# malak29/video-text-detection-system

Measured on AMD Instinct MI355X. Metric: frames/sec (detect+recognize) @720p, 1/2/4/8 MI355X; box IoU vs CPU ref, higher is better.
Workload: dtype f16

## Files before the change

video-text-detection-system_amd/csrc/vtd_api.cpp:

```cpp
#include <algorithm>
#include <cmath>
#include <cstdio>
#include <cstdlib>
#include <cstring>
#include <map>
#include <memory>
#include <string>
#include <vector>

#include "../../include/vtd.h"
#include "vtd_common.h"

int vtd_launch_conv(const ConvParams& p, int cfg, hipStream_t stream);
int vtd_conv_num_configs();
bool vtd_conv_config_valid(const ConvParams& p, int cfg);
int vtd_launch_preprocess(const uint8_t* frames, int n, int H, int W, half_t* out, const int* xb, const int* xk, int ksx,
                          const int* yb, const int* yk, int ksy, int max_rows, hipStream_t stream);
int vtd_launch_nchw_to_input(const float* x, half_t* out, int n, hipStream_t stream);
int vtd_launch_maxpool(const TensorDesc& in, const TensorDesc& out, int n, int kh, int kw, int sh, int sw, int pad_h, int pad_w,
                       hipStream_t stream);
void vtd_stem_pool_pack_weights(const float* w_folded, half_t* packed);
int vtd_launch_stem_pool(const TensorDesc& in, const TensorDesc& out, const half_t* w_packed, const float* bias, int n, hipStream_t stream);
extern "C" int vtd_head_entry_halo_steps(int py, int px, int nch1, int* out);
int vtd_launch_head_entry_halo(const ConvParams& c, const int* steps_dev, int nsteps, int big_tiles, hipStream_t stream);
#ifdef VTD_EXPERIMENTAL_CANDIDATES
extern "C" int vtd_head_entry_half_schedule(const int* steps, int nsteps, int* out);
int vtd_launch_head_entry_half(const ConvParams& c, const int* sched_dev, int nsteps, hipStream_t stream);
int vtd_head_entry_pair_tables(int py, int px, int c2ch, int* half_steps, int* plan);
int vtd_launch_head_entry_pair(const ConvParams& c, const int* half_steps_dev, const int* plan_dev, int nh, hipStream_t stream);
#endif
bool vtd_conv_halo_supported(const ConvParams& c, int* bn_out, int* tw_out);
bool vtd_conv_halo_c64_supported(const ConvParams& c, int tw);
int vtd_launch_conv_halo(const ConvParams& c, int bn, int tw, hipStream_t stream);
bool vtd_pointwise128_supported(const ConvParams& c);
int vtd_launch_pointwise128(const ConvParams& c, hipStream_t stream);
void vtd_head_tail_pack_w1(const half_t* w1_gemm, half_t* packed);
void vtd_head_tail_pack_w2(const float* w2, half_t* packed);
int vtd_launch_head_tail(const TensorDesc& in, const half_t* w1, const float* bias1, const half_t* w2, float b2, float* out, int n,
                         hipStream_t stream);

int vtd_launch_crop_resize(const uint8_t* frames, int H, int W, const int32_t* boxes, int ncrops, uint8_t* out, hipStream_t s);
int vtd_launch_crnn_conv1(const uint8_t* in_u8, const float* in_f32, const half_t* w, const float* bias, half_t* out, int n, hipStream_t s);
int vtd_launch_lstm(const half_t* xs, const half_t* whh, half_t* hout, int D, int T, hipStream_t s);
int vtd_launch_ctc_greedy(const float* logits, int n, int T, int V, int ld, const int32_t* id2char, int blank, int apply_softmax,
                          int32_t* out, hipStream_t s);
int vtd_launch_compact_rows(const float* in, float* out, int64_t rows, int V, int ld, hipStream_t s);
int vtd_dbloss_ws_bytes();
int vtd_launch_dbloss(const float* prob, const float* thresh, const float* prob_t, const float* thresh_t, int64_t n, float smooth, double* workspace,
                      float* out4, double* sums5, hipStream_t stream);
int vtd_launch_dbloss_backward(const float* prob, const float* thresh, const float* prob_t, const float* thresh_t, int64_t n, float smooth,
                               const double* sums5, const float* grad_out4, float* grad_prob, float* grad_thresh, hipStream_t stream);
int vtd_launch_binary_counts(const float* pred, const float* target, int64_t n, float threshold, int64_t* counts4, hipStream_t stream);
int64_t vtd_dbhead_ws_bytes(int n, int H, int W, int backward);
int vtd_launch_dbhead_pack(const void* x, int dtype, int n, int H, int W, void* feats, hipStream_t s);
int vtd_launch_dbhead_forward(const void* feats, int n, int H, int W, const vtd_dbhead_params* params, int training, float momentum, float eps,
                              void* ws, float* prob, float* thresh, float* stats_out, hipStream_t s);
int vtd_launch_dbhead_backward_input(int n, int H, int W, const vtd_dbhead_params* params, void* scratch, float* dfeats, float* dscale, hipStream_t s);
int vtd_launch_dbhead_unpack_input_grad(const float* dfeats, const float* dscale, int n, int H, int W, float* out, hipStream_t s);
int vtd_launch_dbhead_backward(const void* feats, int n, int H, int W, const vtd_dbhead_params* params, int training, const void* ws,
                               const float* prob, const float* thresh, const float* gprob, const float* gthresh, const vtd_dbhead_params* grads,
                               void* scratch, hipStream_t s);

namespace vtd {

enum : int {
    ERR_ARG = -1100,
    ERR_UNKNOWN_KEY = -1101,
    ERR_SHAPE = -1102,
    ERR_MISSING_KEY = -1103,
    ERR_NOT_FINALIZED = -1104,
    ERR_BATCH = -1105,
    ERR_GEOMETRY = -1106,
    ERR_CAPACITY = -1107,
};

using StateDict = std::map<std::string, std::vector<float>>;

struct DeviceArena {
    std::vector<void*> blocks;
    size_t total = 0;
    int alloc(void** out, size_t bytes, bool zero) {
        void* p = nullptr;
        bytes = (bytes + 255) & ~size_t(255);
        hipError_t e = hipMalloc(&p, bytes);
        if (e != hipSuccess) return -(int)e;
        if (zero) {
            e = hipMemset(p, 0, bytes);
            if (e != hipSuccess) return -(int)e;
// ... 6 lines not shown
    ~DeviceArena() {
        for (void* p : blocks) (void)hipFree(p);
    }
};

static TensorDesc make_desc(int n, int h, int w, int c, int ring, int ring_br) {
    TensorDesc t;
    t.ptr = nullptr;
    t.n = n; t.h = h; t.w = w; t.c = c; t.ring = ring;
    t.hp = h + ring + ring_br;
    t.wp = w + ring + ring_br;
    return t;
}

struct ConvOp {
    TensorDesc in, out, res;
    bool has_res = false;
    half_t* w = nullptr;
    half_t* w_panel = nullptr;
    float* bias = nullptr;
    int k_hi_step = 32, cin_steps = 1, kw = 1, s_step = 0, r_step = 0;
    int K = 0, cout = 0, cout_pad = 0, stride = 1, in_y0 = 0, in_x0 = 0, flags = 0, ps_cout = 0, res_shift = 0;
    int ho = 0, wo = 0;
    int64_t macs_per_image = 0;
    void* out_f32 = nullptr;
    int ldc = 0;
    int seg_cols = 0;
    void* seg_out[3] = {nullptr, nullptr, nullptr};
    int seg_ldc[3] = {0, 0, 0};
    const float* head_w = nullptr;
    float head_b = 0.f;
    const uint32_t* plist = nullptr;
    const int* tile_combo = nullptr;
    const uint32_t* plist_b = nullptr;
    const int* tile_combo_border = nullptr;
    int tiles_border = 0;
    const int* he_steps = nullptr;
    int he_nsteps = 0;
    const int* hh_sched = nullptr;
    const int* hp_half_steps = nullptr;
    const int* hp_plan = nullptr;
    int hp_nh = 0;
    const int* tile_combo_b = nullptr;
    int tiles_per_img_b = 0;
    int tiles_per_img = 0, seg1_steps = 0, cin_steps2 = 0, kw2 = 0, s_step2 = 0, r_step2 = 0, img_h = 0, img_w = 0;
    TensorDesc in2;
    const float* bias_tab = nullptr;
    bool dual = false;
    int in2_mul = 1, in2_shr = 0;
    int pool_pw = 0;
};

struct Op {
    enum Kind { CONV, POOL, FINAL, STEMPOOL, HEADTAIL, BORDER } kind;
    ConvOp conv;
    TensorDesc pin, pout;
    int pk[6] = {0, 0, 0, 0, 0, 0};
    const float* fw = nullptr;
    float fbias = 0.f;
    int final_slot = 0;
    const half_t* spw = nullptr;
    const float* spb = nullptr;
    const half_t* htw1 = nullptr;
    const half_t* htw2 = nullptr;
};

static void fill_conv_params(const ConvOp& c, int n, ConvParams& p) {
    std::memset(&p, 0, sizeof(p));
    p.in = c.in.ptr; p.wgt = c.w; p.k_hi_step = c.k_hi_step; p.cin_steps = c.cin_steps; p.kw = c.kw; p.s_step = c.s_step; p.r_step = c.r_step; p.bias = c.bias;
    p.res = c.has_res ? c.res.ptr : nullptr;
    p.out = (c.flags & (EPI_OUT_F32 | EPI_OUT_F16)) ? c.out_f32 : (void*)c.out.ptr;
    p.M = n * c.ho * c.wo; p.K = c.K; p.cout = c.cout; p.cout_pad = c.cout_pad;
    p.ho = c.ho; p.wo = c.wo;
    p.in_hp = c.in.hp; p.in_wp = c.in.wp; p.in_c = c.in.c; p.in_y0 = c.in_y0; p.in_x0 = c.in_x0; p.stride = c.stride;
    p.out_hp = c.out.hp; p.out_wp = c.out.wp; p.out_c = c.out.c; p.out_ring = c.out.ring;
    p.res_hp = c.res.hp; p.res_wp = c.res.wp; p.res_ring = c.res.ring; p.res_shift = c.res_shift;
    p.ps_cout = c.ps_cout; p.flags = c.flags; p.ldc = c.ldc;
    p.seg_cols = c.seg_cols;
    for (int i = 0; i < 3; ++i) { p.seg_out[i] = c.seg_out[i]; p.seg_ldc[i] = c.seg_ldc[i]; }
    p.head_w = c.head_w; p.head_b = c.head_b; p.prob_out = (float*)c.out_f32;
    if (c.plist) {
        p.plist = c.plist; p.tile_combo = c.tile_combo; p.tiles_per_img = c.tiles_per_img;
        p.plist_b = c.plist_b; p.tile_combo_b = c.tile_combo_b; p.tiles_per_img_b = c.tiles_per_img_b;
        p.in2 = c.in2.ptr; p.in2_hp = c.in2.hp; p.in2_wp = c.in2.wp; p.in2_c = c.in2.c; p.in2_ring = c.in2.ring;
        p.seg1_steps = c.seg1_steps; p.cin_steps2 = c.cin_steps2; p.kw2 = c.kw2; p.s_step2 = c.s_step2; p.r_step2 = c.r_step2;
        p.bias_tab = c.bias_tab; p.img_h = c.img_h; p.img_w = c.img_w;
        p.M = n * c.tiles_per_img * 128;
    }
    p.pool_pw = c.pool_pw;
    if (c.dual) {
        p.in2 = c.in2.ptr; p.in2_hp = c.in2.hp; p.in2_wp = c.in2.wp; p.in2_c = c.in2.c; p.in2_ring = c.in2.ring;
        p.in2_mul = c.in2_mul; p.in2_shr = c.in2_shr;
        p.seg1_steps = c.seg1_steps; p.cin_steps2 = c.cin_steps2; p.kw2 = 1; p.s_step2 = 0; p.r_step2 = 0;
    }
}

static const int kHaloCfg = 100;
static const int kHaloC64Cfg = 101;
static const int kHalo64Cfg = 104;
static const int kHeadEntryHalo256Cfg = 103;
static const int kHeadEntryPairCfg = 105;
static const int kPointwiseCfg = 106;
static const int kHeadEntryHalfCfg = 107;
static const int kHeadEntryHaloCfg = 102;
static bool halo_enabled() {
    const char* e = std::getenv("VTD_HALO_CONV");
    return !(e && e[0] == '0');
}

static int pick_tile_height(const ConvParams& p, int table_cfg) {
    if (const char* e = std::getenv("VTD_TILE_HEIGHT_MODEL"); e && e[0] == '0') return table_cfg;
    if (std::getenv("VTD_FORCE_CONV_CFG")) return table_cfg;
    static const struct { int cfg, bm, bn; double eff; } family[5] = {{0, 256, 128, 1.0}, {14, 256, 128, 1.04}, {13, 272, 128, 0.92}, {12, 208, 128, 0.80},
                                                                      {15, 256, 256, 1.07}};
    auto cost_of = [&](int cfg) -> double {
        for (const auto& k : family)
            if (k.cfg == cfg) {
                if (!vtd_conv_config_valid(p, k.cfg)) return 0.0;
                const int64_t tiles = (int64_t)((p.M + k.bm - 1) / k.bm) * (p.cout_pad / k.bn);
                return (double)((tiles + 255) / 256) * k.bm * k.bn / k.eff;
            }
        return 0.0;
    };
    int best = table_cfg;
    double best_cost = cost_of(table_cfg);
    if (best_cost == 0.0) return table_cfg;
    const double keep = best_cost * 0.94;
    double other_cost = keep;
    for (const auto& k : family) {
        if (k.cfg == table_cfg) continue;
        const double c = cost_of(k.cfg);
        if (c > 0.0 && c < other_cost) { other_cost = c; best = k.cfg; }
    }
    (void)best_cost;
    return best;
}

static int launch_conv_op(const ConvOp& c, int n, hipStream_t s, int cfg = -1, float* prob_out = nullptr) {
    ConvParams p;
    fill_conv_params(c, n, p);
    if (prob_out) p.prob_out = prob_out;
#ifdef VTD_EXPERIMENTAL_CANDIDATES
    if (cfg == kHeadEntryPairCfg) {
        if (!c.hp_half_steps || !c.tile_combo_border) return ERR_GEOMETRY;
        return vtd_launch_head_entry_pair(p, c.hp_half_steps, c.hp_plan, c.hp_nh, s);
    }
    if (cfg == kHeadEntryHalfCfg) {
        if (!c.hh_sched || !c.tile_combo_border) return ERR_GEOMETRY;
        return vtd_launch_head_entry_half(p, c.hh_sched, c.he_nsteps, s);
    }
#else
    if (cfg == kHeadEntryPairCfg || cfg == kHeadEntryHalfCfg) return ERR_GEOMETRY;
#endif
    if (cfg == kHeadEntryHaloCfg || cfg == kHeadEntryHalo256Cfg) {
        if (!c.he_steps || !c.tile_combo_border) return ERR_GEOMETRY;
        return vtd_launch_head_entry_halo(p, c.he_steps, c.he_nsteps, cfg == kHeadEntryHalo256Cfg ? 1 : 0, s);
// ... 238 lines not shown
    const char* p = text;
    while (*p) {
        const char* eol = std::strchr(p, '\n');
        std::string line = eol ? std::string(p, eol) : std::string(p);
        p = eol ? eol + 1 : p + line.size();
        if (line.empty() || line[0] == '#') continue;
        const size_t sp = line.find_last_of(" \t");
        if (sp == std::string::npos || sp + 1 >= line.size()) return ERR_ARG;
        char* end = nullptr;
        const long v = std::strtol(line.c_str() + sp + 1, &end, 10);
        if (!end || *end != 0) return ERR_ARG;
        size_t ke = sp;
        while (ke > 0 && (line[ke - 1] == ' ' || line[ke - 1] == '\t')) --ke;
        m->tuning[line.substr(0, ke)] = (int)v;
    }
    return 0;
}

static int64_t get_tuning_text(const ModelBase* m, char* buf, int64_t cap) {
    if (!m) return ERR_ARG;
    std::string out;
    for (const auto& kv : m->tuning) out += kv.first + " " + std::to_string(kv.second) + "\n";
    if (buf && cap > 0) {
        const size_t ncopy = std::min((size_t)cap - 1, out.size());
        std::memcpy(buf, out.data(), ncopy);
        buf[ncopy] = 0;
    }
    return (int64_t)out.size() + 1;
}

static int batch_bucket(int n, int cap) {
    int b = 1;
    while (b < n) b <<= 1;
    return std::min(b, cap);
}

}

struct vtd_detector : vtd::ModelBase {
    std::string backbone;
    int max_batch = 0;
    bool finalized = false;
    std::vector<Op> ops;
    TensorDesc input;
    std::map<std::string, TensorDesc> taps;
    std::map<std::pair<int, int>, PreTables> pre;
    int64_t macs = 0;
    float* final_out[2] = {nullptr, nullptr};
    std::map<int, std::vector<int>> tuned;
    bool head_tail_kernel = true;
    bool fuse_stem_pool = true;
    bool fuse_fpn_head = true;
    bool fuse_downsample = true;
    size_t p2_ops = 0;
    bool profiling = false;
    int prof_only = -1;
    std::vector<hipEvent_t> ev_pool;
    size_t ev_used = 0;
    std::vector<std::pair<int, std::pair<hipEvent_t, hipEvent_t>>> ev_spans;
    std::vector<double> prof_ms;
    std::vector<int64_t> prof_calls;
    std::vector<double> prof_macs;
    hipEvent_t take_event() {
        if (ev_used == ev_pool.size()) {
            hipEvent_t e;
            if (hipEventCreate(&e) != hipSuccess) return nullptr;
            ev_pool.push_back(e);
        }
        return ev_pool[ev_used++];
    }
    ~vtd_detector() {
        for (hipEvent_t e : ev_pool) (void)hipEventDestroy(e);
    }
};


struct vtd_recognizer : vtd::ModelBase {
    int vocab = 0, max_crops = 0;
    bool finalized = false;
    bool fuse_pools = true;
    uint8_t* resized = nullptr;
    half_t* w1 = nullptr;
    float* b1 = nullptr;
    TensorDesc t1;
    std::vector<Op> ops;
    TensorDesc t7, h0, h1;
    ConvOp xs_gemm[2], cls_gemm;
    half_t* whh[2] = {nullptr, nullptr};
    half_t* xs = nullptr;
    float* logits_pad = nullptr;
    std::map<std::string, TensorDesc> taps;
    int64_t macs = 0;
    std::map<int, std::vector<int>> tuned;
};

namespace vtd {

struct Fold {
    std::vector<double> scale, shift;
};

static inline half_t half_of(double v) {
    volatile float f = (float)v;
    return (half_t)f;
}

// ... 489 lines not shown
                TensorDesc t1;
                if ((rc = new_tensor(hout, hout, width, t1))) return rc;
                Fold f1, f2;
                if ((rc = fold_bn(d, pre + ".bn1", "", width, f1))) return rc;
                ConvOp c1;
                if ((rc = build_conv(d, c1, x, t1, pre + ".conv1.weight", f1, cin, width, 3, 3, stride, 1, EPI_RELU))) return rc;
                push_conv(c1);
                if ((rc = new_tensor(hout, hout, width, y, (fuse && st == 0 && b == counts[st] - 1) ? 2 : 1))) return rc;
                if ((rc = fold_bn(d, pre + ".bn2", "", width, f2))) return rc;
                ConvOp c2;
                HostConv h2;
                h2.host_only = fold_ds;
                if ((rc = build_conv(d, c2, t1, y, pre + ".conv2.weight", f2, width, width, 3, 3, 1, 1, fold_ds ? EPI_RELU : (EPI_RELU | EPI_RESIDUAL), &h2))) return rc;
                if (fold_ds) {
                    if ((rc = attach_second_segment(d, c2, h2, ds_op, ds_host, stride, 0))) return rc;
                } else {
                    c2.has_res = true; c2.res = idt; c2.res_shift = 0;
                }
                push_conv(c2);
            } else {
                TensorDesc t1, t2;
                if ((rc = new_tensor(hin, hin, width, t1))) return rc;
                Fold f1, f2, f3;
                if ((rc = fold_bn(d, pre + ".bn1", "", width, f1))) return rc;
                ConvOp c1;
                if ((rc = build_conv(d, c1, x, t1, pre + ".conv1.weight", f1, cin, width, 1, 1, 1, 0, EPI_RELU))) return rc;
                push_conv(c1);
                if ((rc = new_tensor(hout, hout, width, t2))) return rc;
                if ((rc = fold_bn(d, pre + ".bn2", "", width, f2))) return rc;
                ConvOp c2;
                if ((rc = build_conv(d, c2, t1, t2, pre + ".conv2.weight", f2, width, width, 3, 3, stride, 1, EPI_RELU))) return rc;
                push_conv(c2);
                if ((rc = new_tensor(hout, hout, cout, y, (fuse && st == 0 && b == counts[st] - 1) ? 2 : 1))) return rc;
                if ((rc = fold_bn(d, pre + ".bn3", "", cout, f3))) return rc;
                ConvOp c3;
                HostConv h3;
                h3.host_only = fold_ds;
                if ((rc = build_conv(d, c3, t2, y, pre + ".conv3.weight", f3, width, cout, 1, 1, 1, 0, fold_ds ? EPI_RELU : (EPI_RELU | EPI_RESIDUAL), &h3))) return rc;
                if (fold_ds) {
                    if ((rc = attach_second_segment(d, c3, h3, ds_op, ds_host, stride, 0))) return rc;
                } else {
                    c3.has_res = true; c3.res = idt; c3.res_shift = 0;
                }
                push_conv(c3);
            }
            x = y;
            cin = cout;
        }
        tapsC[st] = x;
        d->taps["c" + std::to_string(st + 2)] = x;
    }

    TensorDesc last;
    for (int i = 0; i < (fuse ? 3 : 4); ++i) {
        const TensorDesc& feat = tapsC[3 - i];
        TensorDesc lat;
        if ((rc = new_tensor(feat.h, feat.w, 256, lat))) return rc;
        Fold f;
        const std::string k = "fpn.inner_blocks." + std::to_string(i);
        if ((rc = fold_bn(d, "", k + ".bias", 256, f))) return rc;
        ConvOp c;
        if ((rc = build_conv(d, c, feat, lat, k + ".weight", f, feat.c, 256, 1, 1, 1, 0, i ? EPI_RESIDUAL : 0))) return rc;
        if (i) { c.has_res = true; c.res = last; c.res_shift = 1; }
        push_conv(c);
        last = lat;
    }
    TensorDesc p2;
    if (!fuse) {
        if ((rc = new_tensor(160, 160, 256, p2))) return rc;
        Fold f;
        if ((rc = fold_bn(d, "", "fpn.layer_blocks.3.bias", 256, f))) return rc;
        ConvOp c;
        if ((rc = build_conv(d, c, last, p2, "fpn.layer_blocks.3.weight", f, 256, 256, 3, 3, 1, 1, 0))) return rc;
        push_conv(c);
        d->taps["p2"] = p2;
        d->p2_ops = d->ops.size();
    } else if (!d->get("fpn.inner_blocks.3.weight", (size_t)256 * tapsC[0].c) || !d->get("fpn.layer_blocks.3.weight", (size_t)256 * 256 * 9)) {
        return ERR_MISSING_KEY;
    }
    for (int i = 0; i < 3; ++i) {
        const std::string k = "fpn.layer_blocks." + std::to_string(i);
        if (!d->get(k + ".weight", (size_t)256 * 256 * 9) || !d->get(k + ".bias", 256)) return ERR_MISSING_KEY;
    }

    const char* branch[2] = {"head.probability_head.", "head.threshold_head."};
    for (int br = 0; br < 2; ++br) {
        const std::string hp = branch[br];
        TensorDesc h1;
        if ((rc = new_tensor(160, 160, 64, h1))) return rc;
        Fold f1, f2;
        ConvOp c1;
        if (fuse) {
            if ((rc = build_classed_head_entry(d, c1, tapsC[0], last, h1, hp))) return rc;
        } else {
            if ((rc = fold_bn(d, hp + "1", hp + "0.bias", 64, f1))) return rc;
            if ((rc = build_conv(d, c1, p2, h1, hp + "0.weight", f1, 256, 64, 3, 3, 1, 1, EPI_RELU))) return rc;
        }
        if ((rc = fold_bn(d, hp + "4", hp + "3.bias", 64, f2))) return rc;
        ConvOp c2;
        TensorDesc h2 = make_desc(B, 320, 320, 64, 1, 1);
        std::vector<half_t> w1_host;
        if ((rc = build_convt(d, c2, h1, h2, hp + "3.weight", f2, 64, 64, EPI_RELU, &w1_host))) return rc;
        auto w6 = d->get(hp + "6.weight", 64 * 4), b6 = d->get(hp + "6.bias", 1);
        if (!w6 || !b6) return ERR_MISSING_KEY;
        std::vector<float> wf(4 * 64);
        for (int blk = 0; blk < 4; ++blk)
            for (int ci = 0; ci < 64; ++ci) wf[blk * 64 + ci] = (*w6)[ci * 4 + blk];
        float* wdev = nullptr;
        if ((rc = upload(d->arena, wf.data(), wf.size() * sizeof(float), (void**)&wdev))) return rc;
        c2.flags = EPI_HEAD_FINAL;
        c2.head_w = wdev;
        c2.head_b = (*b6)[0];
        Op o1, o2;
        o1.kind = Op::CONV; o1.conv = c1; o1.final_slot = br;
        o2.kind = Op::FINAL; o2.conv = c2; o2.final_slot = br;
        if (d->head_tail_kernel) {
            std::vector<half_t> p1((size_t)4 * 4 * 2 * 64 * 8), p2((size_t)2 * 64 * 8);
            vtd_head_tail_pack_w1(w1_host.data(), p1.data());
// ... 156 lines not shown
}

int vtd_dbhead_train_backward(const void* feats_dev, int n, int height, int width, const vtd_dbhead_params* params, int training,
                              const void* workspace_dev, const float* prob_dev, const float* thresh_dev, const float* grad_prob_dev,
                              const float* grad_thresh_dev, const vtd_dbhead_params* grads, void* scratch_dev, vtd_stream stream) {
    return vtd_launch_dbhead_backward(feats_dev, n, height, width, params, training, workspace_dev, prob_dev, thresh_dev, grad_prob_dev,
                                      grad_thresh_dev, grads, scratch_dev, (hipStream_t)stream);
}

int vtd_dbhead_train_backward_input(int n, int height, int width, const vtd_dbhead_params* params, void* scratch_dev, float* dfeats_dev,
                                    float* dscale_dev, vtd_stream stream) {
    return vtd_launch_dbhead_backward_input(n, height, width, params, scratch_dev, dfeats_dev, dscale_dev, (hipStream_t)stream);
}

int vtd_dbhead_unpack_input_grad(const float* dfeats_dev, const float* dscale_dev, int n, int height, int width, float* grad_nchw_dev,
                                 vtd_stream stream) {
    return vtd_launch_dbhead_unpack_input_grad(dfeats_dev, dscale_dev, n, height, width, grad_nchw_dev, (hipStream_t)stream);
}

int vtd_device_count(void) {
    int n = 0;
    hipError_t e = hipGetDeviceCount(&n);
    return e == hipSuccess ? n : -(int)e;
}

int vtd_detector_create(const char* backbone, int max_batch, vtd_detector** out) {
    if (!backbone || !out || max_batch <= 0) return ERR_ARG;
    const std::string b = backbone;
    if (b != "resnet18" && b != "resnet50") return ERR_ARG;
    auto* d = new vtd_detector();
    d->backbone = b;
    d->max_batch = max_batch;
    *out = d;
    return 0;
}

void vtd_detector_destroy(vtd_detector* d) { delete d; }

int vtd_detector_set_tensor(vtd_detector* d, const char* key, const float* host_data, int64_t numel) {
    if (!d || !key || !host_data || numel < 0) return ERR_ARG;
    const std::string k = key;
    if (!known_detector_key(k)) return ERR_UNKNOWN_KEY;
    if (k.size() > 19 && k.compare(k.size() - 19, 19, "num_batches_tracked") == 0) return 0;
    d->sd[k].assign(host_data, host_data + numel);
    return 0;
}

int vtd_detector_set_option(vtd_detector* d, const char* name, int value) {
    if (!d || !name || d->finalized) return ERR_ARG;
    if (std::string(name) == "fuse_fpn_head") { d->fuse_fpn_head = value != 0; return 0; }
    if (std::string(name) == "fuse_stem_pool") { d->fuse_stem_pool = value != 0; return 0; }
    if (std::string(name) == "head_tail_kernel") { d->head_tail_kernel = value != 0; return 0; }
    if (std::string(name) == "fuse_downsample") { d->fuse_downsample = value != 0; return 0; }
    return ERR_UNKNOWN_KEY;
}

int vtd_detector_finalize(vtd_detector* d, vtd_stream stream) {
    if (!d) return ERR_ARG;
    if (d->finalized) return ERR_ARG;
    int rc = build_detector_graph(d);
    if (rc) return rc;
    hipError_t e = hipStreamSynchronize((hipStream_t)stream);
    if (e != hipSuccess) return -(int)e;
    d->sd.clear();
    d->finalized = true;
    return 0;
}

int vtd_detector_preprocess(vtd_detector* d, const uint8_t* frames_dev, int n, int height, int width, vtd_stream stream) {
    if (!d || !frames_dev || height <= 0 || width <= 0) return ERR_ARG;
    if (!d->finalized) return ERR_NOT_FINALIZED;
    if (n <= 0 || n > d->max_batch) return ERR_BATCH;
    PreTables t;
    int rc = get_pre_tables(d, height, width, t);
    if (rc) return rc;
    return vtd_launch_preprocess(frames_dev, n, height, width, d->input.ptr, t.xb, t.xk, t.ksx, t.yb, t.yk, t.ksy, t.max_rows,
                                 (hipStream_t)stream);
}

int vtd_detector_set_input_nchw(vtd_detector* d, const float* x_dev, int n, vtd_stream stream) {
    if (!d || !x_dev) return ERR_ARG;
    if (!d->finalized) return ERR_NOT_FINALIZED;
    if (n <= 0 || n > d->max_batch) return ERR_BATCH;
    return vtd_launch_nchw_to_input(x_dev, d->input.ptr, n, (hipStream_t)stream);
}

static int run_detector_ops(vtd_detector* d, int n, float* prob_dev, float* thresh_dev, hipStream_t s, size_t op_end) {
    float* outs[2] = {prob_dev, thresh_dev};
    const int bucket = batch_bucket(n, d->max_batch);
    auto tit = d->tuned.find(bucket);
    if (tit == d->tuned.end()) {
        std::vector<int> cfgs(d->ops.size(), -1);
        for (size_t oi = 0; oi < d->ops.size(); ++oi)
            if (d->ops[oi].kind == Op::CONV) {
                int rc = choose_config(d, d->ops[oi].conv, bucket, s, &cfgs[oi]);
                if (rc) return rc;
            }
        tit = d->tuned.emplace(bucket, std::move(cfgs)).first;
    }
    const std::vector<int>& cfgs = tit->second;
    for (size_t oi = 0; oi < op_end; ++oi) {
        const Op& o = d->ops[oi];
        int rc = 0;
        if (o.final_slot == 1 && !thresh_dev) continue;
        if (o.kind == Op::BORDER && (oi == 0 || (cfgs[oi - 1] != kHeadEntryHaloCfg && cfgs[oi - 1] != kHeadEntryHalo256Cfg && cfgs[oi - 1] != kHeadEntryPairCfg && cfgs[oi - 1] != kHeadEntryHalfCfg)))
            continue;
        hipEvent_t e0 = nullptr, e1 = nullptr;
        const bool prof = d->profiling && (d->prof_only < 0 || d->prof_only == (int)oi);
        if (prof) {
            e0 = d->take_event();
            e1 = d->take_event();
            if (!e0 || !e1) return ERR_ARG;
            VTD_HIP_CHECK(hipEventRecord(e0, s));
        }
        switch (o.kind) {
            case Op::CONV: rc = launch_conv_op(o.conv, n, s, cfgs[oi]); break;
            case Op::POOL: rc = vtd_launch_maxpool(o.pin, o.pout, n, o.pk[0], o.pk[1], o.pk[2], o.pk[3], o.pk[4], o.pk[5], s); break;
            case Op::FINAL: rc = launch_conv_op(o.conv, n, s, 7, outs[o.final_slot]); break;
            case Op::HEADTAIL:
                rc = vtd_launch_head_tail(o.conv.in, o.htw1, o.conv.bias, o.htw2, o.conv.head_b, outs[o.final_slot], n, s);
                break;
            case Op::BORDER: rc = launch_border_tiles(o.conv, n, s); break;
            case Op::STEMPOOL: rc = vtd_launch_stem_pool(o.pin, o.pout, o.spw, o.spb, n, s); break;
        }
        if (rc) return rc;
        if (prof) {
            VTD_HIP_CHECK(hipEventRecord(e1, s));
            d->ev_spans.push_back({(int)oi, {e0, e1}});
            d->prof_macs[oi] += (o.kind != Op::POOL) ? (double)o.conv.macs_per_image * n : 0.0;
        }
    }
    return 0;
}

int vtd_detector_forward(vtd_detector* d, int n, float* prob_dev, float* thresh_dev, vtd_stream stream) {
    if (!d || !prob_dev) return ERR_ARG;
    if (!d->finalized) return ERR_NOT_FINALIZED;
    if (n <= 0 || n > d->max_batch) return ERR_BATCH;
    return run_detector_ops(d, n, prob_dev, thresh_dev, (hipStream_t)stream, d->ops.size());
}

int vtd_detector_forward_features(vtd_detector* d, int n, void* feats_dev, vtd_stream stream) {
    if (!d || !feats_dev) return ERR_ARG;
    if (!d->finalized) return ERR_NOT_FINALIZED;
    if (n <= 0 || n > d->max_batch) return ERR_BATCH;
    if (d->fuse_fpn_head || !d->p2_ops || !d->taps.count("p2")) return -2801;
    if ((uintptr_t)feats_dev & 15) return -2803;
    hipStream_t s = (hipStream_t)stream;
    int rc = run_detector_ops(d, n, nullptr, nullptr, s, d->p2_ops);
    if (rc) return rc;
    const TensorDesc& p2 = d->taps["p2"];
    VTD_HIP_CHECK(hipMemcpyAsync(feats_dev, p2.ptr, (size_t)n * p2.hp * p2.wp * p2.c * sizeof(half_t), hipMemcpyDeviceToDevice, s));
    return 0;
}

int vtd_detector_set_profiling(vtd_detector* d, int enable) {
    if (!d || !d->finalized) return ERR_ARG;
    d->profiling = enable != 0;
    d->prof_only = enable >= 2 ? enable - 2 : -1;
    if (d->prof_only >= (int)d->ops.size()) return ERR_ARG;
    d->ev_spans.clear();
    d->ev_used = 0;
    d->prof_ms.assign(d->ops.size(), 0.0);
    d->prof_calls.assign(d->ops.size(), 0);
    d->prof_macs.assign(d->ops.size(), 0.0);
    return 0;
}

int vtd_detector_num_ops(const vtd_detector* d) { return d ? (int)d->ops.size() : 0; }

int vtd_detector_set_tuning(vtd_detector* d, const char* table_text) {
    if (!d) return ERR_ARG;
    int rc = set_tuning_text(d, table_text);
    if (!rc) d->tuned.clear();
    return rc;
}
// ... 2 lines not shown

int vtd_detector_tuning_measured(const vtd_detector* d) { return d && d->tuning_measured ? 1 : 0; }

int vtd_detector_get_profile(vtd_detector* d, int op_index, char* name, int name_cap, double* total_ms, int64_t* calls,
                             double* total_macs, vtd_stream stream) {
    if (!d || op_index < 0 || op_index >= (int)d->ops.size() || !name || name_cap < 32 || !total_ms || !calls || !total_macs)
        return ERR_ARG;
    if (!d->ev_spans.empty()) {
        hipError_t e = hipStreamSynchronize((hipStream_t)stream);
        if (e != hipSuccess) return -(int)e;
        for (auto& sp : d->ev_spans) {
            float ms = 0.f;
            e = hipEventElapsedTime(&ms, sp.second.first, sp.second.second);
            if (e != hipSuccess) return -(int)e;
            d->prof_ms[sp.first] += ms;
            d->prof_calls[sp.first] += 1;
        }
        d->ev_spans.clear();
        d->ev_used = 0;
    }
    const Op& o = d->ops[op_index];
    if (o.kind == Op::CONV) {
        const ConvOp& c = o.conv;
        static const char* kTile[] = {"256,128,s3", "128,128,s2", "128,128,s3", "256,64,s2", "256,64,s3", "128,64,s2", "128,64,s3",
                                      "64,256,s2", "128,64,s2,classed", "128,64,s3,classed", "256,64,s2,classed", "256,64,s3,classed", "208,128,s3", "272,128,s3", "256,128,s3,16w", "256,256,s2", "128,64,s6"};
        int cfg = -1;
        if (!d->tuned.empty()) cfg = d->tuned.rbegin()->second[op_index];
        if (cfg == kHeadEntryPairCfg)
            std::snprintf(name, name_cap, "head_entry_pair M/img=%d N=%d K=%d (lateral+smooth+head conv composed; border classes in the "
                          "next slot)", c.ho * c.wo, c.cout, c.K);
        else if (cfg == kHeadEntryHalfCfg)
            std::snprintf(name, name_cap, "head_entry_half M/img=%d N=%d K=%d (lateral+smooth+head conv composed, half halos two steps ahead; border classes in the "
                          "next slot)", c.ho * c.wo, c.cout, c.K);
        else if (cfg == kHeadEntryHalo256Cfg)
            std::snprintf(name, name_cap, "head_entry_halo256 M/img=%d N=%d K=%d (lateral+smooth+head conv composed; border classes in the "
                          "next slot)", c.ho * c.wo, c.cout, c.K);
        else if (cfg == kHeadEntryHaloCfg)
            std::snprintf(name, name_cap, "head_entry_halo M/img=%d N=%d K=%d (lateral+smooth+head conv composed; border classes in the "
                          "next slot)", c.ho * c.wo, c.cout, c.K);
        else if (cfg == kPointwiseCfg)
            std::snprintf(name, name_cap, "pointwise128 1x1%s streaming M/img=%d N=%d K=%d", c.has_res ? "+top-down add" : "", c.ho * c.wo, c.cout, c.K);
        else if (cfg == kHaloCfg || cfg == kHaloC64Cfg || cfg == kHalo64Cfg)
            std::snprintf(name, name_cap, "conv_halo%s 3x3 M/img=%d N=%d K=%d", cfg == kHaloC64Cfg ? "_c64_persistent" : cfg == kHalo64Cfg ? "64" : "",
                          c.ho * c.wo, c.cout, c.K);
        else
            std::snprintf(name, name_cap, "conv_igemm<%s> M/img=%d N=%d K=%d%s", (cfg >= 0 && cfg < 17) ? kTile[cfg] : "default",
                          c.ho * c.wo, c.cout, c.K, c.plist ? " (lateral+smooth+head conv composed)" : "");
    } else if (o.kind == Op::POOL) {
        std::snprintf(name, name_cap, "maxpool %dx%d/s%d", o.pk[0], o.pk[1], o.pk[2]);
    } else if (o.kind == Op::BORDER) {
        std::snprintf(name, name_cap, "conv_igemm<128,64,s3,classed> border classes of the composed head entry (%d tiles/img)", o.conv.tiles_border);
    } else if (o.kind == Op::HEADTAIL) {
        std::snprintf(name, name_cap, "head_tail ConvT1+BN+ReLU+ConvT2+sigmoid fused M/img=%d N=256 K=64", o.conv.ho * o.conv.wo);
    } else if (o.kind == Op::STEMPOOL) {
        std::snprintf(name, name_cap, "stem_pool conv7x7/s2+BN+ReLU+maxpool3x3/s2 fused M/img=%d N=64 K=147", 320 * 320);
    } else {
        std::snprintf(name, name_cap, "conv_igemm<64,256,s2> ConvT1+ConvT2+sigmoid fused M/img=%d", o.conv.ho * o.conv.wo);
    }
    const bool have = d->prof_ms.size() == d->ops.size();
    *total_ms = have ? d->prof_ms[op_index] : 0.0;
    *calls = have ? d->prof_calls[op_index] : 0;
    *total_macs = have ? d->prof_macs[op_index] : 0.0;
    return 0;
}

int vtd_detector_read_tap(vtd_detector* d, const char* name, int n, float* host_out, int64_t capacity, vtd_stream stream) {
    if (!d || !name || !host_out) return ERR_ARG;
    if (!d->finalized) return ERR_NOT_FINALIZED;
    auto it = d->taps.find(name);
    if (it == d->taps.end()) return ERR_UNKNOWN_KEY;
    const TensorDesc& t = it->second;
    if (n <= 0 || n > t.n) return ERR_BATCH;
    const int creal = (std::string(name) == "input") ? 3 : t.c;
    if (capacity < (int64_t)n * creal * t.h * t.w) return ERR_CAPACITY;
    return read_tensor_nchw(t, n, creal, host_out, (hipStream_t)stream);
}

int64_t vtd_detector_macs_per_frame(const vtd_detector* d) { return d ? d->macs : 0; }

}

namespace vtd {

static int build_recognizer_graph(vtd_recognizer* r) {
    const int D = r->max_crops;
    int rc;
    auto new_tensor = [&](int h, int w, int c, int ring, TensorDesc& t) {
        t = make_desc(D, h, w, c, ring, ring);
        return r->alloc_tensor(t);
    };
    void* p = nullptr;
    if ((rc = r->arena.alloc(&p, (size_t)D * 32 * 128 * 3, true))) return rc;
    r->resized = (uint8_t*)p;
    {
        Fold f;
        if ((rc = fold_bn(r, "cnn.1", "cnn.0.bias", 64, f))) return rc;
        auto w = r->get("cnn.0.weight", 64 * 3 * 3 * 3);
        if (!w) return ERR_MISSING_KEY;
        std::vector<half_t> wp(64 * 32, (half_t)0.f);
        std::vector<float> bp(64);
        for (int co = 0; co < 64; ++co) {
            bp[co] = (float)f.shift[co];
            for (int c = 0; c < 3; ++c)
                for (int rr = 0; rr < 3; ++rr)
                    for (int ss = 0; ss < 3; ++ss)
                        wp[co * 32 + (rr * 3 + ss) * 3 + c] = half_of((double)(*w)[((co * 3 + c) * 3 + rr) * 3 + ss] * f.scale[co]);
// ... 219 lines not shown
```

Measured before the change: 12700.

## Fuse FPN top-down lateral 1x1 convs C5/C4/C3 into one persistent kernel

Adds a persistent HIP kernel that computes the C5, C4 and C3 lateral 1x1 convolutions with their nearest-upsample residual adds in a single pass. It keeps the intermediate C5 and C4 lateral results in registers instead of writing them out and reading them back between three launches. Inputs stream through a 4-stage global_load_lds pipeline with register-cached weights. At build time the path is chosen per batch bucket by autotuning against the three-launch split, with an env override. It adds register pressure and a fixed 512-block grid.

```diff
diff --git a/video-text-detection-system_amd/csrc/fpn_topdown.hip b/video-text-detection-system_amd/csrc/fpn_topdown.hip
--- /dev/null
+++ b/video-text-detection-system_amd/csrc/fpn_topdown.hip
@@ -0,0 +1,319 @@
+#include "vtd_common.h"
+
+#include <cstring>
+
+namespace {
+
+struct TopdownParams {
+    const half_t *c5, *c4, *c3;
+    const half_t *w5, *w4, *w3;
+    const float *b5, *b4, *b3;
+    half_t* out;
+    int hp5, wp5, r5, hp4, wp4, r4, hp3, wp3, r3, hpo, wpo, ro;
+    int bw, bpi;
+    int items;
+};
+
+template <int N>
+__device__ __forceinline__ void td_wait_vmcnt() { asm volatile("s_waitcnt vmcnt(%0)" ::"n"(N) : "memory"); }
+__device__ __forceinline__ void td_barrier() {
+    __builtin_amdgcn_s_barrier();
+    asm volatile("" ::: "memory");
+}
+
+__device__ __forceinline__ uint32_t td_pack(float a, float b) {
+    const half2v h = {(half_t)a, (half_t)b};
+    uint32_t u = __builtin_bit_cast(uint32_t, h);
+    asm volatile("" : "+v"(u));
+    return u;
+}
+__device__ __forceinline__ float td_lo(uint32_t u) { return (float)__builtin_bit_cast(half2v, u)[0]; }
+__device__ __forceinline__ float td_hi(uint32_t u) { return (float)__builtin_bit_cast(half2v, u)[1]; }
+
+constexpr int TD_NST = 4, TD_STAGE_BYTES = 64 * 256, TD_STAGES_PER_ITEM = 7;
+constexpr int TD_LDS = TD_NST * TD_STAGE_BYTES + 3 * 256 * 4;
+
+__global__ __launch_bounds__(256, 2) void fpn_topdown_kernel(const TopdownParams p) {
+    extern __shared__ __attribute__((aligned(16))) char td_smem[];
+    float* const bias_lds = (float*)(td_smem + TD_NST * TD_STAGE_BYTES);
+    const int tid = threadIdx.x, lane = tid & 63;
+    const int blk = __builtin_amdgcn_readfirstlane(tid >> 6);
+    const int fr = lane & 15, fq = lane >> 4;
+
+    const char* const w5p = (const char*)p.w5 + blk * (16 * 4096);
+    const char* const w4p = (const char*)p.w4 + blk * (8 * 4096);
+    half8 wf[4][4];
+    {
+        const half8* const w3p = (const half8*)p.w3 + (size_t)blk * 4 * 256 + lane;
+#pragma unroll
+        for (int s = 0; s < 4; ++s)
+#pragma unroll
+            for (int i = 0; i < 4; ++i) wf[i][s] = w3p[(s * 4 + i) * 64];
+    }
+    bias_lds[tid] = p.b5[tid];
+    bias_lds[256 + tid] = p.b4[tid];
+    bias_lds[512 + tid] = p.b3[tid];
+    __syncthreads();
+#pragma unroll
+    for (int i = 0; i < 4; ++i)
+#pragma unroll
+        for (int s = 0; s < 4; ++s) asm volatile("" ::"v"(wf[i][s]));
+
+    const int first = blockIdx.x, stride = gridDim.x;
+    if (first >= p.items) return;
+    const int nt = (p.items - first + stride - 1) / stride;
+    const int total = nt * TD_STAGES_PER_ITEM;
+
+    auto item_origin = [&](int item, int& img, int& by, int& bx) {
+        const int it = __builtin_amdgcn_readfirstlane(item);
+        img = it / p.bpi;
+        const int rem = it - img * p.bpi;
+        by = rem / p.bw;
+        bx = rem - by * p.bw;
+    };
+    const int d_px = lane >> 4;
+    const int swz = ((lane & 15) ^ (4 * blk + d_px)) << 3;
+    auto issue = [&](int item, int sidx, int slot) {
+        int img, by, bx;
+        item_origin(item, img, by, bx);
+        const int y5 = 4 * by + blk, x5 = 4 * bx + d_px;
+        char* const dst = td_smem + slot * TD_STAGE_BYTES + blk * 1024;
+        if (sidx == 0) {
+            const half_t* src = p.c5 + (((int64_t)img * p.hp5 + y5 + p.r5) * p.wp5 + x5 + p.r5) * 512 + swz;
+#pragma unroll
+            for (int k = 0; k < 4; ++k)
+                __builtin_amdgcn_global_load_lds((const VTD_AS1 void*)(src + 128 * k), (VTD_AS3 void*)(dst + 4096 * k), 16, 0, 0);
+        } else if (sidx < 3) {
+            const half_t* src = p.c4 + (((int64_t)img * p.hp4 + 2 * y5 + p.r4) * p.wp4 + 2 * x5 + p.r4) * 256 + 128 * (sidx - 1) + swz;
+#pragma unroll
+            for (int k = 0; k < 4; ++k)
+                __builtin_amdgcn_global_load_lds((const VTD_AS1 void*)(src + ((k >> 1) * p.wp4 + (k & 1)) * 256),
+                                                 (VTD_AS3 void*)(dst + 4096 * k), 16, 0, 0);
+        } else {
+            const int g = sidx - 3;
+            const int y4 = 2 * y5 + (g >> 1), x4 = 2 * x5 + (g & 1);
+            const half_t* src = p.c3 + (((int64_t)img * p.hp3 + 2 * y4 + p.r3) * p.wp3 + 2 * x4 + p.r3) * 128 + swz;
+#pragma unroll
+            for (int k = 0; k < 4; ++k)
+                __builtin_amdgcn_global_load_lds((const VTD_AS1 void*)(src + ((k >> 1) * p.wp3 + (k & 1)) * 128),
+                                                 (VTD_AS3 void*)(dst + 4096 * k), 16, 0, 0);
+        }
+    };
+    int issued = 0, nik = 0, nis = 0;
+    auto issue_next = [&]() {
+        if (issued < total) {
+            issue(first + nik * stride, nis, issued & (TD_NST - 1));
+            ++issued;
+            if (++nis == TD_STAGES_PER_ITEM) { nis = 0; ++nik; }
+        }
+    };
+    auto wait_stage = [&](int g) {
+        const int younger = issued - g - 1;
+        if (younger >= 2) td_wait_vmcnt<8>();
+        else if (younger == 1) td_wait_vmcnt<4>();
+        else td_wait_vmcnt<0>();
+    };
+    auto lds_frag = [&](const char* sb, int j, int s) { return *(const half8*)(sb + (j * 16 + fr) * 256 + (((4 * s + fq) ^ fr) << 4)); };
+
+    issue_next();
+    issue_next();
+    issue_next();
+    wait_stage(0);
+
+    for (int k = 0; k < nt; ++k) {
+        const int g0 = k * TD_STAGES_PER_ITEM;
+        int img, by, bx;
+        item_origin(first + k * stride, img, by, bx);
+        half8 wq[24][4];
+        uint32_t woff = lane * 16;
+        asm volatile("" : "+v"(woff));
+        auto wload = [&](int u) {
+            const char* src = u < 16 ? w5p + u * 4096 : w4p + (u - 16) * 4096;
+#pragma unroll
+            for (int i = 0; i < 4; ++i) wq[u][i] = *(const half8*)(src + woff + i * 1024);
+        };
+        auto wprefetch = [&](int t) {
+            if (t + 4 < 16) wload(t + 4);
+            if (t + 2 >= 16 && t + 2 < 24) wload(t + 2);
+        };
+#pragma unroll
+        for (int u = 0; u < 4; ++u) wload(u);
+
+        td_barrier();
+        uint32_t l5[4][2];
+        {
+            const char* sb = td_smem + ((g0 + 0) & (TD_NST - 1)) * TD_STAGE_BYTES;
+            floatx4 acc[4];
+#pragma unroll
+            for (int i = 0; i < 4; ++i) acc[i] = floatx4{0.f, 0.f, 0.f, 0.f};
+#pragma unroll
+            for (int t = 0; t < 16; ++t) {
+                wprefetch(t);
+                const half8 af = lds_frag(sb, t >> 2, t & 3);
+#pragma unroll
+                for (int i = 0; i < 4; ++i) acc[i] = __builtin_amdgcn_mfma_f32_16x16x32_f16(wq[t][i], af, acc[i], 0, 0, 0);
+                __builtin_amdgcn_sched_barrier(0);
+            }
+            wait_stage(g0 + 1);
+#pragma unroll
+            for (int i = 0; i < 4; ++i) {
+                const floatx4 b = *(const floatx4*)(bias_lds + 64 * blk + 32 * (i >> 1) + 8 * fq + 4 * (i & 1));
+                l5[i][0] = td_pack(acc[i][0] + b[0], acc[i][1] + b[1]);
+                l5[i][1] = td_pack(acc[i][2] + b[2], acc[i][3] + b[3]);
+            }
+        }
+
+        uint32_t l4[4][4][2];
+        {
+            floatx4 acc[4][4];
+#pragma unroll
+            for (int i = 0; i < 4; ++i)
+#pragma unroll
+                for (int j = 0; j < 4; ++j) acc[i][j] = floatx4{0.f, 0.f, 0.f, 0.f};
+#pragma unroll
+            for (int hs = 0; hs < 2; ++hs) {
+                td_barrier();
+                const char* sb = td_smem + ((g0 + 1 + hs) & (TD_NST - 1)) * TD_STAGE_BYTES;
+#pragma unroll
+                for (int s = 0; s < 4; ++s) {
+                    const int t = 16 + 4 * hs + s;
+                    wprefetch(t);
+                    if (hs == 1 && s == 2) {
+                        issue_next();
+                        issue_next();
+                        issue_next();
+                    }
+                    half8 af[4];
+#pragma unroll
+                    for (int j = 0; j < 4; ++j) af[j] = lds_frag(sb, j, s);
+#pragma unroll
+                    for (int j = 0; j < 4; ++j)
+#pragma unroll
+                        for (int i = 0; i < 4; ++i) acc[i][j] = __builtin_amdgcn_mfma_f32_16x16x32_f16(wq[t][i], af[j], acc[i][j], 0, 0, 0);
+                    __builtin_amdgcn_sched_barrier(0);
+                }
+                wait_stage(g0 + 2 + hs);
+            }
+#pragma unroll
+            for (int i = 0; i < 4; ++i) {
+                const floatx4 b = *(const floatx4*)(bias_lds + 256 + 64 * blk + 32 * (i >> 1) + 8 * fq + 4 * (i & 1));
+#pragma unroll
+                for (int j = 0; j < 4; ++j) {
+                    float v[4];
+#pragma unroll
+                    for (int e = 0; e < 4; ++e) {
+                        v[e] = acc[i][j][e] + b[e];
+                        v[e] += (e & 1) ? td_hi(l5[i][e >> 1]) : td_lo(l5[i][e >> 1]);
+                    }
+                    l4[i][j][0] = td_pack(v[0], v[1]);
+                    l4[i][j][1] = td_pack(v[2], v[3]);
+                }
+            }
+        }
+
+        int fro = fr, fqo = fq;
+        asm volatile("" : "+v"(fro), "+v"(fqo));
+        half_t* const o_lane = p.out + (((int64_t)img * p.hpo + 16 * by + 4 * (fro >> 2) + p.ro) * p.wpo + 16 * bx + 4 * (fro & 3) + p.ro) * 256 + 64 * blk + 8 * fqo;
+#pragma unroll
+        for (int g = 0; g < 4; ++g) {
+            td_barrier();
+            issue_next();
+            const char* sb = td_smem + ((g0 + 3 + g) & (TD_NST - 1)) * TD_STAGE_BYTES;
+            floatx4 acc[4][4];
+#pragma unroll
+            for (int i = 0; i < 4; ++i)
+#pragma unroll
+                for (int j = 0; j < 4; ++j) acc[i][j] = floatx4{0.f, 0.f, 0.f, 0.f};
+            half8 af[2][4];
+#pragma unroll
+            for (int j = 0; j < 4; ++j) af[0][j] = lds_frag(sb, j, 0);
+#pragma unroll
+            for (int s = 0; s < 4; ++s) {
+                if (s < 3) {
+#pragma unroll
+                    for (int j = 0; j < 4; ++j) af[(s + 1) & 1][j] = lds_frag(sb, j, s + 1);
+                }
+#pragma unroll
+                for (int j = 0; j < 4; ++j)
+#pragma unroll
+                    for (int i = 0; i < 4; ++i) acc[i][j] = __builtin_amdgcn_mfma_f32_16x16x32_f16(wf[i][s], af[s & 1][j], acc[i][j], 0, 0, 0);
+                __builtin_amdgcn_sched_barrier(0);
+            }
+            if (g0 + 4 + g < total) wait_stage(g0 + 4 + g);
+#pragma unroll
+            for (int kk = 0; kk < 2; ++kk) {
+                const floatx4 b0 = *(const floatx4*)(bias_lds + 512 + 64 * blk + 32 * kk + 8 * fq), b1 = *(const floatx4*)(bias_lds + 512 + 64 * blk + 32 * kk + 8 * fq + 4);
+#pragma unroll
+                for (int j = 0; j < 4; ++j) {
+                    half8 hv;
+#pragma unroll
+                    for (int e = 0; e < 4; ++e) {
+                        float v0 = acc[2 * kk][j][e] + b0[e], v1 = acc[2 * kk + 1][j][e] + b1[e];
+                        v0 += (e & 1) ? td_hi(l4[2 * kk][g][e >> 1]) : td_lo(l4[2 * kk][g][e >> 1]);
+                        v1 += (e & 1) ? td_hi(l4[2 * kk + 1][g][e >> 1]) : td_lo(l4[2 * kk + 1][g][e >> 1]);
+                        hv[e] = (half_t)v0;
+                        hv[4 + e] = (half_t)v1;
+                    }
+                    const int dy = 2 * (g >> 1) + (j >> 1), dx = 2 * (g & 1) + (j & 1);
+                    *(half8*)(o_lane + (dy * p.wpo + dx) * 256 + 32 * kk) = hv;
+                }
+            }
+        }
+    }
+    td_wait_vmcnt<0>();
+}
+
+}
+
+void vtd_fpn_topdown_pack_weights(const half_t* w, int K, half_t* packed) {
+    const int steps = K / 32;
+    for (int blk = 0; blk < 4; ++blk)
+        for (int s = 0; s < steps; ++s)
+            for (int i = 0; i < 4; ++i)
+                for (int lane = 0; lane < 64; ++lane) {
+                    const int fr = lane & 15, fq = lane >> 4;
+                    const int ch = 64 * blk + 32 * (i >> 1) + 8 * (fr >> 2) + 4 * (i & 1) + (fr & 3);
+                    std::memcpy(packed + ((((size_t)blk * steps + s) * 4 + i) * 64 + lane) * 8, w + (size_t)ch * K + 32 * s + 8 * fq, 8 * sizeof(half_t));
+                }
+}
+
+static bool td_lateral_ok(const ConvParams& c, int cin, bool res) {
+    return !c.plist && !c.in2 && !c.pool_pw && c.K == cin && c.in_c == cin && c.cin_steps * 64 == cin && c.cout == 256 && c.out_c == 256 && c.kw == 1 &&
+           c.stride == 1 && c.in_y0 == c.in_x0 && c.flags == (res ? EPI_RESIDUAL : 0) && (!res || (c.res && c.res_shift == 1)) && c.ho > 0 && c.wo > 0 &&
+           c.M % (c.ho * c.wo) == 0;
+}
+
+bool vtd_fpn_topdown_supported(const ConvParams& c5, const ConvParams& c4, const ConvParams& c3) {
+    if (!td_lateral_ok(c5, 512, false) || !td_lateral_ok(c4, 256, true) || !td_lateral_ok(c3, 128, true)) return false;
+    if ((c5.ho & 3) || (c5.wo & 3) || c4.ho != 2 * c5.ho || c4.wo != 2 * c5.wo || c3.ho != 2 * c4.ho || c3.wo != 2 * c4.wo) return false;
+    const int n = c5.M / (c5.ho * c5.wo);
+    if (n <= 0 || c4.M != n * c4.ho * c4.wo || c3.M != n * c3.ho * c3.wo) return false;
+    if (c4.res != (const half_t*)c5.out || c3.res != (const half_t*)c4.out) return false;
+    if (c4.res_hp != c5.out_hp || c4.res_wp != c5.out_wp || c3.res_hp != c4.out_hp || c3.res_wp != c4.out_wp) return false;
+    return (int64_t)n * (c5.ho / 4) * (c5.wo / 4) < (1 << 30);
+}
+
+int vtd_launch_fpn_topdown(const ConvParams& c5, const ConvParams& c4, const ConvParams& c3, const half_t* packed, hipStream_t stream) {
+    if (!vtd_fpn_topdown_supported(c5, c4, c3) || !packed) return -2501;
+    TopdownParams p;
+    p.c5 = c5.in; p.c4 = c4.in; p.c3 = c3.in;
+    p.w5 = packed; p.w4 = packed + 256 * 512; p.w3 = packed + 256 * (512 + 256);
+    p.b5 = c5.bias; p.b4 = c4.bias; p.b3 = c3.bias;
+    p.out = (half_t*)c3.out;
+    p.hp5 = c5.in_hp; p.wp5 = c5.in_wp; p.r5 = c5.in_y0;
+    p.hp4 = c4.in_hp; p.wp4 = c4.in_wp; p.r4 = c4.in_y0;
+    p.hp3 = c3.in_hp; p.wp3 = c3.in_wp; p.r3 = c3.in_y0;
+    p.hpo = c3.out_hp; p.wpo = c3.out_wp; p.ro = c3.out_ring;
+    p.bw = c5.wo / 4; p.bpi = (c5.ho / 4) * p.bw;
+    p.items = c5.M / (c5.ho * c5.wo) * p.bpi;
+    const int grid = p.items < 512 ? p.items : 512;
+    static bool attr_set = false;
+    if (!attr_set) {
+        hipError_t e = hipFuncSetAttribute((const void*)fpn_topdown_kernel, hipFuncAttributeMaxDynamicSharedMemorySize, TD_LDS);
+        if (e != hipSuccess) return -(int)e;
+        attr_set = true;
+    }
+    hipLaunchKernelGGL(fpn_topdown_kernel, dim3(grid), dim3(256), TD_LDS, stream, p);
+    hipError_t e = hipGetLastError();
+    return e == hipSuccess ? 0 : -(int)e;
+}
diff --git a/video-text-detection-system_amd/csrc/vtd_api.cpp b/video-text-detection-system_amd/csrc/vtd_api.cpp
--- a/video-text-detection-system_amd/csrc/vtd_api.cpp
+++ b/video-text-detection-system_amd/csrc/vtd_api.cpp
@@ -34,6 +34,9 @@
 int vtd_launch_conv_halo(const ConvParams& c, int bn, int tw, hipStream_t stream);
 bool vtd_pointwise128_supported(const ConvParams& c);
 int vtd_launch_pointwise128(const ConvParams& c, hipStream_t stream);
+void vtd_fpn_topdown_pack_weights(const half_t* w, int K, half_t* packed);
+bool vtd_fpn_topdown_supported(const ConvParams& c5, const ConvParams& c4, const ConvParams& c3);
+int vtd_launch_fpn_topdown(const ConvParams& c5, const ConvParams& c4, const ConvParams& c3, const half_t* packed, hipStream_t stream);
 void vtd_head_tail_pack_w1(const half_t* w1_gemm, half_t* packed);
 void vtd_head_tail_pack_w2(const float* w2, half_t* packed);
 int vtd_launch_head_tail(const TensorDesc& in, const half_t* w1, const float* bias1, const half_t* w2, float b2, float* out, int n,
@@ -146,7 +149,7 @@
 };
 
 struct Op {
-    enum Kind { CONV, POOL, FINAL, STEMPOOL, HEADTAIL, BORDER } kind;
+    enum Kind { CONV, POOL, FINAL, STEMPOOL, HEADTAIL, BORDER, TOPDOWN } kind;
     ConvOp conv;
     TensorDesc pin, pout;
     int pk[6] = {0, 0, 0, 0, 0, 0};
@@ -157,6 +160,7 @@
     const float* spb = nullptr;
     const half_t* htw1 = nullptr;
     const half_t* htw2 = nullptr;
+    const half_t* tdw = nullptr;
 };
 
 static void fill_conv_params(const ConvOp& c, int n, ConvParams& p) {
@@ -196,6 +200,8 @@
 static const int kHeadEntryPairCfg = 105;
 static const int kPointwiseCfg = 106;
 static const int kHeadEntryHalfCfg = 107;
+static const int kTopdownFusedCfg = 108;
+static const int kTopdownSplitCfg = 109;
 static const int kHeadEntryHaloCfg = 102;
 static bool halo_enabled() {
     const char* e = std::getenv("VTD_HALO_CONV");
@@ -540,6 +546,8 @@
     bool fuse_stem_pool = true;
     bool fuse_fpn_head = true;
     bool fuse_downsample = true;
+    bool fuse_topdown = true;
+    int td_op = -1;
     size_t p2_ops = 0;
     bool profiling = false;
     int prof_only = -1;
@@ -1135,6 +1143,7 @@
     }
 
     TensorDesc last;
+    HostConv lat_host[4];
     for (int i = 0; i < (fuse ? 3 : 4); ++i) {
         const TensorDesc& feat = tapsC[3 - i];
         TensorDesc lat;
@@ -1143,10 +1152,31 @@
         const std::string k = "fpn.inner_blocks." + std::to_string(i);
         if ((rc = fold_bn(d, "", k + ".bias", 256, f))) return rc;
         ConvOp c;
-        if ((rc = build_conv(d, c, feat, lat, k + ".weight", f, feat.c, 256, 1, 1, 1, 0, i ? EPI_RESIDUAL : 0))) return rc;
+        if ((rc = build_conv(d, c, feat, lat, k + ".weight", f, feat.c, 256, 1, 1, 1, 0, i ? EPI_RESIDUAL : 0, &lat_host[i]))) return rc;
         if (i) { c.has_res = true; c.res = last; c.res_shift = 1; }
         push_conv(c);
         last = lat;
+    }
+    if (fuse && d->fuse_topdown) {
+        const size_t at = d->ops.size();
+        ConvParams q[3];
+        for (int i = 0; i < 3; ++i) fill_conv_params(d->ops[at - 3 + i].conv, B, q[i]);
+        if (vtd_fpn_topdown_supported(q[0], q[1], q[2])) {
+            std::vector<half_t> packed((size_t)256 * (512 + 256 + 128));
+            size_t off = 0;
+            for (int i = 0; i < 3; ++i) {
+                vtd_fpn_topdown_pack_weights(lat_host[i].w.data(), lat_host[i].K, packed.data() + off);
+                off += (size_t)256 * lat_host[i].K;
+            }
+            Op o;
+            o.kind = Op::TOPDOWN;
+            if ((rc = upload(d->arena, packed.data(), packed.size() * sizeof(half_t), (void**)&o.tdw))) return rc;
+            o.conv = d->ops[at - 1].conv;
+            o.conv.macs_per_image = 0;
+            for (int i = 0; i < 3; ++i) o.conv.macs_per_image += d->ops[at - 3 + i].conv.macs_per_image;
+            d->td_op = (int)at;
+            d->ops.push_back(o);
+        }
     }
     TensorDesc p2;
     if (!fuse) {
@@ -1409,6 +1439,7 @@
     if (std::string(name) == "fuse_stem_pool") { d->fuse_stem_pool = value != 0; return 0; }
     if (std::string(name) == "head_tail_kernel") { d->head_tail_kernel = value != 0; return 0; }
     if (std::string(name) == "fuse_downsample") { d->fuse_downsample = value != 0; return 0; }
+    if (std::string(name) == "fuse_topdown") { d->fuse_topdown = value != 0; return 0; }
     return ERR_UNKNOWN_KEY;
 }
 
@@ -1440,6 +1471,61 @@
     if (!d->finalized) return ERR_NOT_FINALIZED;
     if (n <= 0 || n > d->max_batch) return ERR_BATCH;
     return vtd_launch_nchw_to_input(x_dev, d->input.ptr, n, (hipStream_t)stream);
+}
+
+static int launch_topdown(const vtd_detector* d, int n, hipStream_t s) {
+    ConvParams q[3];
+    for (int i = 0; i < 3; ++i) fill_conv_params(d->ops[d->td_op - 3 + i].conv, n, q[i]);
+    return vtd_launch_fpn_topdown(q[0], q[1], q[2], d->ops[d->td_op].tdw, s);
+}
+
+static int choose_topdown(vtd_detector* d, int n, hipStream_t s, const std::vector<int>& cfgs, int* choice) {
+    const Op& o = d->ops[d->td_op];
+    const ConvOp& c5 = d->ops[d->td_op - 3].conv;
+    char buf[160];
+    std::snprintf(buf, sizeof buf, "topdown|in%dx%dx%d+%d+%d|out%dx%d|co%d|n%d", c5.in.h, c5.in.w, c5.in.c, d->ops[d->td_op - 2].conv.in.c, o.conv.in.c,
+                  o.conv.ho, o.conv.wo, o.conv.cout, n);
+    const std::string key = buf;
+    if (const char* f = std::getenv("VTD_FORCE_TOPDOWN"); f && (f[0] == '0' || f[0] == '1')) {
+        *choice = f[0] == '1' ? kTopdownFusedCfg : kTopdownSplitCfg;
+        return 0;
+    }
+    auto it = d->tuning.find(key);
+    if (it != d->tuning.end() && (it->second == kTopdownFusedCfg || it->second == kTopdownSplitCfg)) {
+        *choice = it->second;
+        return 0;
+    }
+    *choice = kTopdownFusedCfg;
+    if (!autotune_enabled()) return 0;
+    hipEvent_t e0, e1;
+    VTD_HIP_CHECK(hipEventCreate(&e0));
+    VTD_HIP_CHECK(hipEventCreate(&e1));
+    auto split = [&]() {
+        int r = 0;
+        for (int i = 0; i < 3 && !r; ++i) r = launch_conv_op(d->ops[d->td_op - 3 + i].conv, n, s, cfgs[d->td_op - 3 + i]);
+        return r;
+    };
+    float ms[2] = {0.f, 0.f};
+    int rc = 0;
+    for (int which = 0; which < 2 && !rc; ++which) {
+        auto run = [&]() { return which ? launch_topdown(d, n, s) : split(); };
+        if ((rc = run())) break;
+        (void)hipEventRecord(e0, s);
+        for (int rep = 0; rep < 3 && !rc; ++rep) rc = run();
+        (void)hipEventRecord(e1, s);
+        if (hipEventSynchronize(e1) != hipSuccess) rc = ERR_ARG;
+        (void)hipEventElapsedTime(&ms[which], e0, e1);
+    }
+    (void)hipEventDestroy(e0);
+    (void)hipEventDestroy(e1);
+    if (rc) return rc;
+    *choice = ms[1] < ms[0] ? kTopdownFusedCfg : kTopdownSplitCfg;
+    if (const char* v = std::getenv("VTD_AUTOTUNE_VERBOSE"); v && v[0] == '1')
+        std::fprintf(stderr, "[autotune] FPN top-down n=%d: three lateral launches %.1f us, fused launch %.1f us -> %s\n", n, ms[0] / 3.f * 1e3f,
+                     ms[1] / 3.f * 1e3f, *choice == kTopdownFusedCfg ? "fused" : "three launches");
+    d->tuning[key] = *choice;
+    d->tuning_measured = true;
+    return 0;
 }
 
 static int run_detector_ops(vtd_detector* d, int n, float* prob_dev, float* thresh_dev, hipStream_t s, size_t op_end) {
@@ -1453,6 +1539,10 @@
                 int rc = choose_config(d, d->ops[oi].conv, bucket, s, &cfgs[oi]);
                 if (rc) return rc;
             }
+        if (d->td_op >= 0) {
+            int rc = choose_topdown(d, bucket, s, cfgs, &cfgs[d->td_op]);
+            if (rc) return rc;
+        }
         tit = d->tuned.emplace(bucket, std::move(cfgs)).first;
     }
     const std::vector<int>& cfgs = tit->second;
@@ -1462,6 +1552,10 @@
         if (o.final_slot == 1 && !thresh_dev) continue;
         if (o.kind == Op::BORDER && (oi == 0 || (cfgs[oi - 1] != kHeadEntryHaloCfg && cfgs[oi - 1] != kHeadEntryHalo256Cfg && cfgs[oi - 1] != kHeadEntryPairCfg && cfgs[oi - 1] != kHeadEntryHalfCfg)))
             continue;
+        if (d->td_op >= 0) {
+            const bool fused_td = cfgs[d->td_op] == kTopdownFusedCfg;
+            if (fused_td ? ((int)oi >= d->td_op - 3 && (int)oi < d->td_op) : (int)oi == d->td_op) continue;
+        }
         hipEvent_t e0 = nullptr, e1 = nullptr;
         const bool prof = d->profiling && (d->prof_only < 0 || d->prof_only == (int)oi);
         if (prof) {
@@ -1479,6 +1573,7 @@
                 break;
             case Op::BORDER: rc = launch_border_tiles(o.conv, n, s); break;
             case Op::STEMPOOL: rc = vtd_launch_stem_pool(o.pin, o.pout, o.spw, o.spb, n, s); break;
+            case Op::TOPDOWN: rc = launch_topdown(d, n, s); break;
         }
         if (rc) return rc;
         if (prof) {
@@ -1587,6 +1682,9 @@
         std::snprintf(name, name_cap, "conv_igemm<128,64,s3,classed> border classes of the composed head entry (%d tiles/img)", o.conv.tiles_border);
     } else if (o.kind == Op::HEADTAIL) {
         std::snprintf(name, name_cap, "head_tail ConvT1+BN+ReLU+ConvT2+sigmoid fused M/img=%d N=256 K=64", o.conv.ho * o.conv.wo);
+    } else if (o.kind == Op::TOPDOWN) {
+        std::snprintf(name, name_cap, "fpn_topdown C5+C4+C3 laterals fused M/img=%d N=%d K=%d+%d+%d", o.conv.ho * o.conv.wo, o.conv.cout,
+                      d->ops[op_index - 3].conv.K, d->ops[op_index - 2].conv.K, d->ops[op_index - 1].conv.K);
     } else if (o.kind == Op::STEMPOOL) {
         std::snprintf(name, name_cap, "stem_pool conv7x7/s2+BN+ReLU+maxpool3x3/s2 fused M/img=%d N=64 K=147", 320 * 320);
     } else {
```

After: 12670. No clear change (-0.3%).
